# mlvlab/UP-NeRF

Hardware: AMD Instinct MI355X
Metric: training rays/sec (higher is better)
Workload: dtype f32 (f16x3 emulated: 3 fp16 MFMAs per product, fp32 accumulate); 1 GPU; BASELINE.json configs[1]: Brandenburg Gate shape, 4096 rays/GPU/step, 64 coarse + 128 fine samples, two 8x256 fields + candidate/colour heads + TransientNet + appearance/candidate embeddings (763 images), pose optimisation ON, full step incl. both Adam updates; rays_per_gpu=4096, n_images=763, N_samples=64, N_importance=128, parallelism=dp1, field=f16x3

## Files before the change

include/upnerf_hip.h:

```cpp
#ifndef UPNERF_HIP_H
#define UPNERF_HIP_H

#include <stdint.h>

#ifdef __cplusplus
extern "C" {
#endif

#define UPNERF_ABI_VERSION 11
#define UPNERF_EINVAL (-1)
#define UPNERF_EUNSUP (-2)

#ifndef UPNERF_TILE_ROWS
#define UPNERF_TILE_ROWS 64
#endif
#define UPNERF_X0 64
#define UPNERF_AUXK 80
#define UPNERF_CK 16
#define UPNERF_MAX_D 8

int upnerf_abi_version(void);

int upnerf_pose_rays_fwd(int R, const float* se3, const float* c2w, const float* dirs,
                         float* rays_o, float* rays_d, void* stream);
// ... 164 lines not shown
  const float* x0; const float* h; const float* g1; const float* g2; const float* r1;
  const uint64_t* hmask;
  float* gmax;
  float* gz_h;
  float* gz_e;
  float* gz_g1; float* gz_g2;
  float* gz_r1;
  float* dpre_sig_s;
  float* dpre_sig_c;
  float* dpre_rgb;
  float* dxyz;
  const void* PT16;
  const int32_t* wexp;
  int32_t planes;
  int32_t tile_rows;
  uint16_t* gz16;
  int32_t* gzexp;
  void* xs;
  float* tile_part;
  int32_t gz_rg_ld;
  int32_t reserved_;
  const float* wnorm;
  uint16_t* gz_rg16;
  int32_t* gzrgexp;
  uint16_t* gz_g2_16;
  int32_t* gzg2exp;
  uint8_t* gz_lo8;
  int64_t rows_capacity;
} upnerf_field_bwd_args;

#define UPNERF_TILE_PART_STRIDE 1288
int upnerf_tile_part_finish(int R, int S, const float* tile_part, float* rs_g1, float* rs_r1, float* d_wcsig, float* d_bcsig,
                            float* d_wr2, float* d_br2, float* scratch, void* stream);

#define UPNERF_RR_PART_STRIDE 512
int upnerf_ray_part_finish(int R, int S, const float* tile_part, float* rs_g1, float* rs_r1, void* stream);

int upnerf_field_bwd(const upnerf_layout* L, const upnerf_field_bwd_args* a, void* stream);
int upnerf_field_bwd_f16x3(const upnerf_layout* L, const upnerf_field_bwd_args* a, void* stream);

int upnerf_wgrad(int M, const float* A, int lda, int N, const float* B, int ldb, int K,
                 float* dW, int ldo, float* db, float* slabs, int nsplit, void* stream);

#define UPNERF_MAX_WGRAD_GROUPS 32
typedef struct {
  const float* A;
  const float* B;
  float* dW;
  float* db;
  int32_t M, N, K, lda, ldb, ldo;
} upnerf_wgrad_group;
int upnerf_wgrad_grouped_scratch(const upnerf_wgrad_group* groups, int ngroups, int nsplit);
int upnerf_wgrad_grouped(const upnerf_wgrad_group* groups, int ngroups, float* scratch, int nsplit, void* stream);

typedef struct {
  int32_t R; float beta_min;
  const float* feat;
  const float* t_emb;
  const float* w0; const float* b0;
  const float* w1; const float* b1;
  const float* w2; const float* b2;
  const float* w3; const float* b3;
  const float* wf; const float* bf;
  const float* wt; const float* bt;
  const float* wa; const float* ba;
  const float* wb; const float* bb;
  const float* wr; const float* br;
  float* h;
  float* e;
  float* t;
  float* alpha; float* rgb; float* beta;
  float* spre;
} upnerf_transient_args;
typedef struct {
  const float* d_alpha; const float* d_rgb; const float* d_beta;
  float* dz_heads;
  float* gz_t;
  float* gz_e;
  float* gz_h;
  float* g_temb;
  float* g_feat;
} upnerf_transient_grads;
int upnerf_transient_fwd(const upnerf_transient_args* a, void* stream);
int upnerf_transient_bwd(const upnerf_transient_args* a, const upnerf_transient_grads* g, void* stream);

enum {
  UPNERF_WG_F32 = 0,
  UPNERF_WG_F16_TILE,
  UPNERF_WG_F16_FRAG,
  UPNERF_WG_F24,
  UPNERF_WG_PLANES
};
typedef struct {
  const void* p;
  const void* lo;
  const int32_t* exp;
  int32_t ld, kind;
} upnerf_wgrad_operand;

typedef struct {
  const float* slabs; const float* bslabs;
  float* dW; float* db;
  int32_t N, K, TN, TK, nsplit, ldo, rblocks;
  int32_t n2;
  float* dW2; float* db2;
  int32_t ldo2, pad;
// ... 506 lines not shown
```

upnerf_amd/_lib.py:

```python
from __future__ import annotations

import ctypes as C
import os

import torch

from .pass_plan import (AUXK, CK, RR_PART_STRIDE, TILE_PART_STRIDE, WG_F16_FRAG, WG_F16_TILE, WG_F24, WG_F32,
                        WG_PLANES, X0)

_HERE = os.path.dirname(os.path.abspath(__file__))
LIB_PATH = os.environ.get("UPNERF_LIB") or os.path.join(_HERE, "libupnerf_hip.so")
MAX_D = 8

_fp = C.c_void_p


class Layout(C.Structure):
    _fields_ = [("W", C.c_int32), ("D", C.c_int32), ("skip", C.c_int32),
                ("w", C.c_int32 * MAX_D), ("b", C.c_int32 * MAX_D),
                ("we", C.c_int32), ("be", C.c_int32), ("wsig", C.c_int32), ("bsig", C.c_int32),
                ("wc1", C.c_int32), ("bc1", C.c_int32), ("wc2", C.c_int32), ("bc2", C.c_int32),
                ("wcsig", C.c_int32), ("bcsig", C.c_int32), ("wr1", C.c_int32), ("br1", C.c_int32),
                ("wr2", C.c_int32), ("br2", C.c_int32), ("total", C.c_int32),
                ("t_w", C.c_int32 * MAX_D), ("t_skipx", C.c_int32), ("t_we", C.c_int32), ("t_head", C.c_int32),
# ... 307 lines not shown
    _fields_ = [("R", C.c_int32), ("n_tables", C.c_int32), ("hit", _fp), ("t0", _fp), ("t1", _fp), ("rays", _fp), ("rays_c", _fp),
                ("index", _fp), ("count", _fp), ("scratch", _fp), ("tables", PathTable * PATH_MAX_TABLES)]


class OccScatterArgs(C.Structure):
    _fields_ = [("R", C.c_int32), ("n_hit", C.c_int32), ("background", C.c_float), ("reserved_", C.c_int32), ("index", _fp),
                ("rays", _fp), ("rgb_c", _fp), ("depth_c", _fp), ("rgb", _fp), ("depth", _fp)]


class DensityGradArgs(C.Structure):
    _fields_ = [("M", C.c_int32), ("reserved_", C.c_int32), ("points", _fp), ("P", _fp), ("PT", _fp), ("wk_xyz", C.c_float * 10),
                ("sigma", _fp), ("grad", _fp)]


class NormalCompositeArgs(C.Structure):
    _fields_ = [("R", C.c_int32), ("S", C.c_int32), ("grad", _fp), ("w", _fp), ("normal", _fp)]


class VizNormalsArgs(C.Structure):
    _fields_ = [("H", C.c_int32), ("W", C.c_int32), ("n", _fp), ("rot", _fp), ("rgb", _fp)]


class Rng(C.Structure):
    _fields_ = [("seed", C.c_uint64), ("step", C.c_int32), ("row0", C.c_int32), ("row_stride", C.c_int32), ("step_dev", _fp)]


_i, _f, _p = C.c_int, C.c_float, C.c_void_p
_SIGNATURES = {
    "upnerf_abi_version": [],
    "upnerf_pose_rays_fwd": [_i, _p, _p, _p, _p, _p, _p],
    "upnerf_pose_rays_bwd": [_i, _p, _p, _p, _p, _p, _p, _p],
    "upnerf_sample_coarse": [_i, _i, _p, _p, _p, _f, _i, _p, _p],
    "upnerf_uniform_keyed": [_i, _i, C.c_uint64, _i, _p, _i, _i, _i, _p, _p],
    "upnerf_sample_pdf": [_i, _i, _p, _p, _p, _i, _i, _p, _i, _p],
    "upnerf_sort_rows": [_i, _i, _p, _p],
    "upnerf_sample_coarse_keyed": [_i, _i, _p, _p, C.POINTER(Rng), _f, _i, _p, _p],
    "upnerf_resample_sort": [_i, _i, _p, _p, _i, _i, _p, _i, _p, _i, _i, _p, _i, _i, C.POINTER(Rng), _p, _p],
    "upnerf_ray_aux": [_i, _p, _p, C.POINTER(C.c_float), _p, _p, _p],
    "upnerf_field_fwd": [C.POINTER(Layout), C.POINTER(FieldFwdArgs), _p],
    "upnerf_composite_fwd": [C.POINTER(CompositeFwdArgs), _p],
    "upnerf_composite_bwd": [C.POINTER(CompositeBwdArgs), _p],
    "upnerf_field_bwd": [C.POINTER(Layout), C.POINTER(FieldBwdArgs), _p],
    "upnerf_field_fwd_f16x3": [C.POINTER(Layout), C.POINTER(FieldFwdArgs), _p],
    "upnerf_field_bwd_f16x3": [C.POINTER(Layout), C.POINTER(FieldBwdArgs), _p],
    "upnerf_frag16": [_p, _p, _p, C.POINTER(Frag16Desc), _i, C.POINTER(Frag16Desc), _i, _p, _p, _i, _i, _p, _p],
    "upnerf_wgrad": [_i, _p, _i, _i, _p, _i, _i, _p, _i, _p, _p, _i, _p],
    "upnerf_wgrad16_scratch": [C.POINTER(WgradDesc)],
    "upnerf_wgrad16": [C.POINTER(WgradDesc), C.POINTER(WgradPending), _p],
    "upnerf_wgrad_finish": [_p, _p],
    "upnerf_transient_fwd": [_p, _p],
    "upnerf_transient_bwd": [_p, _p, _p],
    "upnerf_wgrad_grouped_scratch": [C.POINTER(WgradGroup), _i, _i],
    "upnerf_wgrad_grouped": [C.POINTER(WgradGroup), _i, _p, _i, _p],
    "upnerf_vec_wgrad": [_i, _p, _i, _i, _p, _i, _i, _p, _p, _p, _i, _p],
    "upnerf_matvec": [_i, _i, _p, _i, _p, _p, _p, _i, _p],
    "upnerf_matvec_rank1": [_i, _i, _p, _i, _p, _p, _p, _i, _p, _p],
    "upnerf_add_pairs": [C.POINTER(AddPair), _i, _p],
    "upnerf_zero": [_p, C.c_longlong, _p],
    "upnerf_vec_wgrad_frag16": [_i, _p, _i, _i, _p, _p, _i, _p, _p, _p, _i, _p],
    "upnerf_ray_sum": [_i, _i, _p, _i, _p, _p],
    "upnerf_ray_part_finish": [_i, _i, _p, _p, _p, _p],
    "upnerf_tile_part_finish": [_i, _i, _p, _p, _p, _p, _p, _p, _p, _p, _p],
    "upnerf_ray_geom_bwd": [_i, _i, _p, _p, _p, _p, _p],
    "upnerf_pack": [_p, C.POINTER(PackDesc), _i, _i, _p],
    "upnerf_gather_rays": [C.POINTER(GatherRaysArgs), _p],
    "upnerf_embed_bwd": [_i, _i, _i, _p, _p, _p, _p],
    "upnerf_embed_bwd_grouped": [_i, _i, _p, C.POINTER(EmbedGroup), _i, _p],
    "upnerf_embed_fwd_grouped": [_i, _i, _p, C.POINTER(EmbedRowsGroup), _i, _p],
    "upnerf_linear": [_i, _i, _i, _p, _i, _p, _i, _p, _p, _i, _i, _p],
    "upnerf_loss_fwd": [C.POINTER(LossArgs), _p, _p, _p, _p],
    "upnerf_loss_bwd": [C.POINTER(LossArgs), _p, C.POINTER(LossGrads), _p],
    "upnerf_frag_copy": [_p, _p, C.POINTER(FragDesc), _i, _p],
    "upnerf_adam": [C.c_int64, _p, _p, _p, _p, _f, _f, _f, _f, _f, _p, _p],
    "upnerf_adam_gather": [_p, _p, _p, _p, _i, _f, _f, _f, _f, _f, _p, _p],
    "upnerf_set_scalars": [_p, _i, C.POINTER(C.c_float), _p],
    "upnerf_scale_exponents": [_p, _i, _p, _p],
    "upnerf_ssim_scratch": [C.POINTER(SsimArgs)],
    "upnerf_ssim": [C.POINTER(SsimArgs), _p, _p],
    "upnerf_conv2d": [C.POINTER(Conv2dArgs), _p],
    "upnerf_maxpool2d": [C.POINTER(Maxpool2dArgs), _p],
    "upnerf_lpips_dist": [C.POINTER(LpipsDistArgs), _p, _p],
    "upnerf_lpips_scratch": [C.POINTER(LpipsScratchArgs)],
    "upnerf_scene_rays": [C.POINTER(SceneRaysArgs), C.POINTER(SceneImage), _p, _p],
    "upnerf_resize_scratch": [C.POINTER(ResizeArgs)],
    "upnerf_resize_linear": [C.POINTER(ResizeArgs), C.POINTER(ResizeMap), _p, _p],
    "upnerf_viz_minmax_scratch": [C.c_longlong],
    "upnerf_viz_minmax": [_p, C.c_longlong, C.c_longlong, _p, _p, _p],
    "upnerf_viz_depth_scratch": [C.POINTER(VizDepthArgs)],
    "upnerf_viz_depth": [C.POINTER(VizDepthArgs), _p, _p],
    "upnerf_viz_pca_scratch": [C.POINTER(VizPcaArgs)],
    "upnerf_viz_pca": [C.POINTER(VizPcaArgs), _p, _p],
    "upnerf_viz_rgb": [C.POINTER(VizRgbArgs), _p],
    "upnerf_path_poses": [C.POINTER(PathPosesArgs), _p],
    "upnerf_path_rays": [C.POINTER(PathRaysArgs), _p],
    "upnerf_grid_columns": [C.POINTER(GridColumnsArgs), _p],
    "upnerf_mtet_scratch": [_i, _i, _i],
    "upnerf_mtet_count": [C.POINTER(MtetArgs), _p, _p, _p],
    "upnerf_mtet_emit": [C.POINTER(MtetArgs), _p, _p],
    "upnerf_occ_words": [_i, _i, _i],
    "upnerf_occ_build_scratch": [_i, _i, _i],
    "upnerf_occ_build": [C.POINTER(OccBuildArgs), _p],
    "upnerf_occ_spans": [C.POINTER(OccSpansArgs), _p],
    "upnerf_occ_compact_scratch": [_i],
    "upnerf_occ_compact": [C.POINTER(OccCompactArgs), _p],
    "upnerf_occ_scatter": [C.POINTER(OccScatterArgs), _p],
    "upnerf_density_grad": [C.POINTER(Layout), C.POINTER(DensityGradArgs), _p],
# ... 69 lines not shown
```

upnerf_amd/csrc/gemm.hip:

```cpp
#include "common.cuh"
#include "wgrad_host.h"

using namespace upnerf_host;

namespace {

template <int MTW, int NTW>
__device__ __forceinline__ void wgrad_tile(int N, int K, const float* __restrict__ A, int lda,
                                           const float* __restrict__ B, int ldb, float* __restrict__ slab,
                                           float* __restrict__ bslab, int mbeg, int mend, int nblk, int kblk) {
  constexpr int TN = 64 * MTW, TK = 64 * NTW;
  constexpr int A4 = WG_CHUNK * TN / 4 / NTHREADS, B4 = WG_CHUNK * TK / 4 / NTHREADS;
  __shared__ __attribute__((aligned(16))) float As[2][WG_CHUNK * TN];
  __shared__ __attribute__((aligned(16))) float Bs[2][WG_CHUNK * TK];
  const int tid = threadIdx.x, lane = tid & 63, wave = tid >> 6;
  const int li = lane & 31, hh = lane >> 5;
  const int n0 = (wave >> 1) * 32 * MTW, k0 = (wave & 1) * 32 * NTW;
  f32x16 acc[MTW][NTW];
  acc_zero(acc);
  float bsum[MTW];
#pragma unroll
  for (int mt = 0; mt < MTW; ++mt) bsum[mt] = 0.f;

  f32x4 ra[A4 > 0 ? A4 : 1], rb[B4 > 0 ? B4 : 1];
// ... 69 lines not shown
      }
  if (bslab && (wave & 1) == 0) {
#pragma unroll
    for (int mt = 0; mt < MTW; ++mt) {
      const float s = bsum[mt] + __shfl_xor(bsum[mt], 32);
      if (hh == 0) bslab[n0 + 32 * mt + li] = s;
    }
  }
}

template <int MTW, int NTW>
__global__ __launch_bounds__(NTHREADS, 1) void wgrad_kernel(int M, int N, int K, const float* __restrict__ A, int lda,
                                                            const float* __restrict__ B, int ldb,
                                                            float* __restrict__ slabs, float* __restrict__ bslabs,
                                                            int rows_per_split) {
  constexpr int TN = 64 * MTW, TK = 64 * NTW;
  const int split = blockIdx.x;
  const int mbeg = split * rows_per_split;
  const int mend = (mbeg + rows_per_split < M) ? mbeg + rows_per_split : M;
  const size_t blk = ((size_t)split * gridDim.y + blockIdx.y) * gridDim.z + blockIdx.z;
  wgrad_tile<MTW, NTW>(N, K, A, lda, B, ldb, slabs + blk * TN * TK,
                       (bslabs && blockIdx.z == 0) ? bslabs + ((size_t)split * gridDim.y + blockIdx.y) * TN : nullptr, mbeg,
                       mend, blockIdx.y * TN, blockIdx.z * TK);
}

struct WgradGroups {
  upnerf_wgrad_group g[UPNERF_MAX_WGRAD_GROUPS];
  int tile_start[UPNERF_MAX_WGRAD_GROUPS + 1];
  int red_start[UPNERF_MAX_WGRAD_GROUPS + 1];
  int n;
};
#define GT 128

__device__ __forceinline__ int find_group(const int* start, int n, int idx) {
  int g = 0;
  while (g + 1 < n && idx >= start[g + 1]) ++g;
  return g;
}

__global__ __launch_bounds__(NTHREADS, 1) void wgrad_grouped_kernel(WgradGroups T, float* __restrict__ slabs,
                                                                    float* __restrict__ bslabs, int nsplit) {
  const int tile = blockIdx.y, split = blockIdx.x;
  const int gi = find_group(T.tile_start, T.n, tile);
  const upnerf_wgrad_group& G = T.g[gi];
  const int gz = (G.K + GT - 1) / GT, local = tile - T.tile_start[gi], by = local / gz, bz = local - by * gz;
  const int rows = (((G.M + nsplit - 1) / nsplit) + WG_CHUNK - 1) / WG_CHUNK * WG_CHUNK;
  const int mbeg = split * rows;
  const int mend = (mbeg + rows < G.M) ? mbeg + rows : G.M;
  const size_t blk = (size_t)tile * nsplit + split;
  wgrad_tile<2, 2>(G.N, G.K, G.A, G.lda, G.B, G.ldb, slabs + blk * GT * GT,
                   (G.db && bz == 0) ? bslabs + blk * GT : nullptr, mbeg < mend ? mbeg : mend, mend, by * GT, bz * GT);
}

__global__ __launch_bounds__(NTHREADS) void wgrad_grouped_reduce_kernel(WgradGroups T, const float* __restrict__ slabs,
                                                                       const float* __restrict__ bslabs, int nsplit) {
  const int gi = find_group(T.red_start, T.n, blockIdx.x);
  const upnerf_wgrad_group& G = T.g[gi];
  const int b = blockIdx.x - T.red_start[gi];
  const int K4 = G.K >> 2, gz = (G.K + GT - 1) / GT;
  const int q = b * NTHREADS + threadIdx.x;
  if (q < G.N * K4) {
    const int n = q / K4, k = (q - n * K4) * 4;
    const int by = n / GT, bz = k / GT;
    const float* src = slabs + ((size_t)(T.tile_start[gi] + by * gz + bz) * nsplit) * GT * GT + (size_t)(n - by * GT) * GT +
                       (k - bz * GT);
    f32x4 s0 = {0.f, 0.f, 0.f, 0.f}, s1 = s0, s2 = s0, s3 = s0;
    int sp = 0;
    for (; sp + 4 <= nsplit; sp += 4) {
      const f32x4 a = *(const f32x4*)&src[(size_t)sp * GT * GT], c = *(const f32x4*)&src[(size_t)(sp + 1) * GT * GT];
      const f32x4 d = *(const f32x4*)&src[(size_t)(sp + 2) * GT * GT], e = *(const f32x4*)&src[(size_t)(sp + 3) * GT * GT];
      s0 += a; s1 += c; s2 += d; s3 += e;
    }
    for (; sp < nsplit; ++sp) s0 += *(const f32x4*)&src[(size_t)sp * GT * GT];
    *(f32x4*)&G.dW[(size_t)n * G.ldo + k] = (s0 + s1) + (s2 + s3);
  }
  if (G.db && q < G.N) {
    const int by = q / GT;
    const float* src = bslabs + ((size_t)(T.tile_start[gi] + by * gz) * nsplit) * GT + (q - by * GT);
    float p0 = 0.f, p1 = 0.f, p2 = 0.f, p3 = 0.f;
    int sp = 0;
    for (; sp + 4 <= nsplit; sp += 4) {
      p0 += src[(size_t)sp * GT]; p1 += src[(size_t)(sp + 1) * GT];
      p2 += src[(size_t)(sp + 2) * GT]; p3 += src[(size_t)(sp + 3) * GT];
    }
    for (; sp < nsplit; ++sp) p0 += src[(size_t)sp * GT];
    G.db[q] = (p0 + p1) + (p2 + p3);
  }
}

__global__ __launch_bounds__(RED_THREADS) void wgrad_reduce_kernel(upnerf_wgrad_pending P) {
  __shared__ f32x4 part[RED_RG][64];
  wgrad_reduce_body(blockIdx.x, threadIdx.x, P, part);
}

template <int K>
__global__ __launch_bounds__(NTHREADS) void vec_wgrad_kernel(int M, const float* __restrict__ v, int ldv, int nvec,
                                                            const float* __restrict__ X, int ldx,
                                                            float* __restrict__ part, int rows_per_split) {
  constexpr int CPR = K / 4, RG = NTHREADS / CPR;
  __shared__ float red[RG][3][K + 4];
  const int tid = threadIdx.x, c4 = tid % CPR, rg = tid / CPR, split = blockIdx.x;
  const int mbeg = split * rows_per_split;
  const int mend = (mbeg + rows_per_split < M) ? mbeg + rows_per_split : M;
  f32x4 acc[3];
  float bacc[3] = {0.f, 0.f, 0.f};
#pragma unroll
  for (int c = 0; c < 3; ++c) acc[c] = f32x4{0.f, 0.f, 0.f, 0.f};
  constexpr int U = 8;
  for (int m = mbeg + rg; m < mend; m += U * RG) {
    f32x4 x[U];
    float vv[U][3];
#pragma unroll
    for (int u = 0; u < U; ++u) {
      const int mm = m + u * RG;
      const bool ok = mm < mend;
      const int mc = ok ? mm : mend - 1;
      x[u] = NT_LOAD((const f32x4*)&X[(size_t)mc * ldx + 4 * c4]);
#pragma unroll
      for (int c = 0; c < 3; ++c) vv[u][c] = (c < nvec) ? v[(size_t)mc * ldv + c] : 0.f;
      if (!ok) {
        x[u] = f32x4{0.f, 0.f, 0.f, 0.f};
#pragma unroll
        for (int c = 0; c < 3; ++c) vv[u][c] = 0.f;
      }
    }
#pragma unroll
    for (int u = 0; u < U; ++u)
#pragma unroll
      for (int c = 0; c < 3; ++c) {
        acc[c].x += vv[u][c] * x[u].x; acc[c].y += vv[u][c] * x[u].y;
        acc[c].z += vv[u][c] * x[u].z; acc[c].w += vv[u][c] * x[u].w;
        bacc[c] += vv[u][c];
      }
  }
#pragma unroll
  for (int c = 0; c < 3; ++c) {
    *(f32x4*)&red[rg][c][4 * c4] = acc[c];
    if (c4 == 0) red[rg][c][K] = bacc[c];
  }
// ... 523 lines not shown
#pragma unroll
        for (int u = 0; u < 8; ++u) {
          const int m = m0 + 16 * u;
          const int mc = m < M ? m : M - 1;
          a[u] = A[(size_t)mc * lda + k];
          xv[u] = m < M ? x[mc] : 0.0f;
        }
#pragma unroll
        for (int u = 0; u < 8; ++u) s += a[u] * xv[u];
        if (R1) {
          const float vk = v1[k];
#pragma unroll
          for (int u = 0; u < 8; ++u) {
            const int m = m0 + 16 * u;
            if (m < M) R1[(size_t)m * ldr + k] += xv[u] * vk;
          }
        }
      }
    }
    part[p][c] = s;
    __syncthreads();
    if (p == 0 && k < K) {
      float t = 0.0f;
#pragma unroll
      for (int q = 0; q < 16; ++q) t += part[q][c];
      y[k] = t + (add ? add[k] : 0.0f);
    }
    return;
  }
  const int m = blockIdx.x * 4 + (threadIdx.x >> 6), lane = threadIdx.x & 63;
  if (m >= M) return;
  float s = 0.0f;
  for (int k = lane; k < K; k += 64) s += A[(size_t)m * lda + k] * x[k];
#pragma unroll
  for (int d = 32; d >= 1; d >>= 1) s += __shfl_xor(s, d);
  if (lane == 0) y[m] = s + (add ? add[m] : 0.0f);
}
extern "C" int upnerf_matvec(int M, int K, const float* A, int lda, const float* x, const float* add, float* y, int trans,
                             void* stream) {
  if (M <= 0 || K <= 0 || !A || !x || !y || lda < K) return UPNERF_EINVAL;
  const int blocks = trans ? (K + 15) / 16 : (M + 3) / 4;
  hipLaunchKernelGGL(matvec_kernel, dim3(blocks), dim3(256), 0, (hipStream_t)stream, M, K, A, lda, x, add, y, trans);
  return (int)hipGetLastError();
}

extern "C" int upnerf_matvec_rank1(int M, int K, const float* A, int lda, const float* x, float* y, float* R, int ldr, const float* v,
                                   void* stream) {
  if (M <= 0 || K <= 0 || !A || !x || !y || !R || !v || lda < K || ldr < K) return UPNERF_EINVAL;
  hipLaunchKernelGGL(matvec_kernel, dim3((K + 15) / 16), dim3(256), 0, (hipStream_t)stream, M, K, A, lda, x, (const float*)nullptr, y, 1, R,
                     ldr, v);
  return (int)hipGetLastError();
}

extern "C" int upnerf_wgrad_grouped_scratch(const upnerf_wgrad_group* groups, int ngroups, int nsplit) {
  if (!groups || ngroups <= 0 || ngroups > UPNERF_MAX_WGRAD_GROUPS || nsplit <= 0) return UPNERF_EINVAL;
  long long tiles = 0;
  for (int j = 0; j < ngroups; ++j)
    tiles += (long long)((groups[j].N + GT - 1) / GT) * ((groups[j].K + GT - 1) / GT);
  const long long n = tiles * nsplit * (GT * GT + GT);
  return n > 0x7fffffffLL ? UPNERF_EUNSUP : (int)n;
}

extern "C" int upnerf_wgrad_grouped(const upnerf_wgrad_group* groups, int ngroups, float* scratch, int nsplit,
                                    void* stream) {
  if (!groups || ngroups <= 0 || ngroups > UPNERF_MAX_WGRAD_GROUPS || !scratch || nsplit <= 0) return UPNERF_EINVAL;
  WgradGroups T;
  T.n = ngroups;
  T.tile_start[0] = T.red_start[0] = 0;
  for (int j = 0; j < ngroups; ++j) {
    const upnerf_wgrad_group& q = groups[j];
    if (!q.A || !q.B || !q.dW || q.M <= 0 || q.N <= 0 || q.K <= 0 || (q.N & 3) || (q.K & 3) || (q.lda & 3) || (q.ldb & 3) ||
        (q.ldo & 3))
      return UPNERF_EINVAL;
    T.g[j] = q;
    T.tile_start[j + 1] = T.tile_start[j] + ((q.N + GT - 1) / GT) * ((q.K + GT - 1) / GT);
    int rb = (q.N * (q.K / 4) + NTHREADS - 1) / NTHREADS;
    if (rb * NTHREADS < q.N) rb = (q.N + NTHREADS - 1) / NTHREADS;
    T.red_start[j + 1] = T.red_start[j] + rb;
  }
  const int tiles = T.tile_start[ngroups];
  float* bslabs = scratch + (size_t)tiles * nsplit * GT * GT;
  hipStream_t st = (hipStream_t)stream;
  hipLaunchKernelGGL(wgrad_grouped_kernel, dim3(nsplit, tiles), dim3(NTHREADS), 0, st, T, scratch, bslabs, nsplit);
  int rc = (int)hipGetLastError();
  if (rc) return rc;
  hipLaunchKernelGGL(wgrad_grouped_reduce_kernel, dim3(T.red_start[ngroups]), dim3(NTHREADS), 0, st, T, scratch, bslabs,
                     nsplit);
  return (int)hipGetLastError();
}

extern "C" int upnerf_vec_wgrad(int M, const float* v, int ldv, int nvec, const float* X, int ldx, int K, float* dw,
                                float* dbv, float* scratch, int nsplit, void* stream) {
  if (M <= 0 || nvec <= 0 || nvec > 4 || K <= 0 || K > 256 || !v || !X || !dw || !scratch || nsplit <= 0)
    return UPNERF_EINVAL;
  hipStream_t st = (hipStream_t)stream;
  const int rows = (M + nsplit - 1) / nsplit;
  if (nvec > 3 || (ldx & 3)) return UPNERF_EINVAL;
  if (K == 256) hipLaunchKernelGGL(vec_wgrad_kernel<256>, dim3(nsplit), dim3(NTHREADS), 0, st, M, v, ldv, nvec, X, ldx, scratch, rows);
  else if (K == 128) hipLaunchKernelGGL(vec_wgrad_kernel<128>, dim3(nsplit), dim3(NTHREADS), 0, st, M, v, ldv, nvec, X, ldx, scratch, rows);
  else if (K == 64) hipLaunchKernelGGL(vec_wgrad_kernel<64>, dim3(nsplit), dim3(NTHREADS), 0, st, M, v, ldv, nvec, X, ldx, scratch, rows);
  else if (K == 32) hipLaunchKernelGGL(vec_wgrad_kernel<32>, dim3(nsplit), dim3(NTHREADS), 0, st, M, v, ldv, nvec, X, ldx, scratch, rows);
  else return UPNERF_EUNSUP;
  int rc = (int)hipGetLastError();
  if (rc) return rc;
  const int total = nvec * (K + 1);
  hipLaunchKernelGGL(vec_wgrad_reduce_kernel, dim3((total + 255) / 256), dim3(256), 0, st, nvec, K, nsplit, scratch, dw,
                     dbv);
  return (int)hipGetLastError();
}

#define TP_STRIDE UPNERF_TILE_PART_STRIDE
#define TP_WCOLS 520
#define TP_NS 128
namespace {
__device__ __forceinline__ void tile_part_rays_body(int idx, int which, int R, int S, const float* __restrict__ part,
                                                    float* __restrict__ rs_g1, float* __restrict__ rs_r1) {
  float* __restrict__ out = which == 0 ? rs_g1 : rs_r1;
  if (idx >= R * 32 || !out) return;
  const int r = idx >> 5, g = idx & 31;
  const long long b = (long long)r * S, e = b + S - 1;
  const int t0 = (int)(b / 64), t1 = (int)(e / 64);
  const int base = TP_WCOLS + (which == 0 ? 0 : 384) + 4 * g;
  f32x4 s = {0.f, 0.f, 0.f, 0.f};
  for (int t = t0; t <= t1; ++t) {
    const int j = r - (int)(((long long)t * 64) / S);
    s += *(const f32x4*)&part[(size_t)t * TP_STRIDE + base + 128 * j];
  }
  *(f32x4*)&out[(size_t)r * 128 + 4 * g] = s;
}
// ... 277 lines not shown
```

upnerf_amd/ops.py:

```python
from __future__ import annotations

import contextlib
import ctypes as C
import os
from typing import Dict, NamedTuple, Optional, Tuple

import torch
import torch.nn.functional as F

from . import _lib
from ._lib import check, lib, ptr, stream

_WS: Dict[Tuple[str, int], torch.Tensor] = {}


class KernelTimer:

    def __init__(self):
        self.enabled = False
        self.only = None
        self.records = {}

    def run(self, name: str, fn, units: int = 0):
        if not self.enabled or (self.only is not None and name not in self.only):
            return fn()
        e0, e1 = torch.cuda.Event(enable_timing=True), torch.cuda.Event(enable_timing=True)
        e0.record()
        out = fn()
        e1.record()
        self.records.setdefault(name, []).append((e0, e1, units))
        return out

    def reset(self):
        self.records = {}

    def summary(self):
        torch.cuda.synchronize()
        out = {}
        for name, evs in self.records.items():
            ms = [a.elapsed_time(b) for a, b, _ in evs]
            out[name] = dict(launches=len(ms), total_ms=sum(ms), avg_ms=sum(ms) / len(ms),
                             units_per_launch=sum(u for _, _, u in evs) / len(evs))
        return out


TIMER = KernelTimer()


def workspace(tag: str, numel: int, device) -> torch.Tensor:
    key = (tag, device.index if device.index is not None else torch.cuda.current_device())
    t = _WS.get(key)
    if t is None or t.numel() < numel:
        t = torch.empty(max(numel, 1), device=device, dtype=torch.float32)
        _WS[key] = t
    return t


def nsplit_for(M: int) -> int:
    return max(1, min(256, M // 64))


def wgrad_into(M: int, A: torch.Tensor, lda: int, N: int, B: torch.Tensor, ldb: int, K: int, dW_ptr: int, ldo: int,
               db_ptr: Optional[int], device, a_off: int = 0, b_off: int = 0):
    ns = nsplit_for(M)
    ws = workspace("wgrad", ns * (256 * 256 + 256), device)
    rc = TIMER.run(f"wgrad_{N}x{K}", lambda: lib.upnerf_wgrad(M, A.data_ptr() + 4 * a_off, lda, N,
                                                              B.data_ptr() + 4 * b_off, ldb, K, dW_ptr, ldo, db_ptr,
                                                              ptr(ws), ns, stream()), units=M)
    check(rc, "upnerf_wgrad")


def wgrad_blocks_into(M: int, A: torch.Tensor, lda: int, N: int, B: torch.Tensor, ldb: int, K: int, dW_ptr: int, ldo: int,
                      db_ptr: Optional[int], device, a_off: int = 0, b_off: int = 0):
    g = _lib.WgradGroup(A=A.data_ptr() + 4 * a_off, B=B.data_ptr() + 4 * b_off, dW=dW_ptr, db=db_ptr, M=M, N=N, K=K, lda=lda,
                        ldb=ldb, ldo=ldo)
    arr = (_lib.WgradGroup * 1)(g)
    nsplit = max(1, min(_DeferredWgrads.NSPLIT, M // 64))
    n = lib.upnerf_wgrad_grouped_scratch(arr, 1, nsplit)
    if n < 0:
        check(n, "upnerf_wgrad_grouped_scratch")
    ws = workspace("wgrad_blocks", n, device)
    check(TIMER.run(f"wgrad_blocks_{N}x{K}", lambda: lib.upnerf_wgrad_grouped(arr, 1, ptr(ws), nsplit, stream())),
          "upnerf_wgrad_grouped")


class _DeferredWgrads:

    enabled = __import__("os").environ.get("UPNERF_DEFER_WGRADS", "1") != "0"
    check_adopted = __import__("os").environ.get("UPNERF_CHECK_DEFERRED", "0") == "1"
    MAX_M = 16384
    NSPLIT = 64

    def __init__(self):
        self.groups, self.keep, self.owners = [], [], []

    def clear(self):
        self.groups, self.keep, self.owners = [], [], []

    def add(self, M, gy, lda, N, x, ldb, K, gw, gb, owners=()):
        self.owners += [(p, t.data_ptr()) for p, t in owners if t is not None]
        torch.autograd.Variable._execution_engine.queue_callback(self.flush)
        self.groups.append(_lib.WgradGroup(A=gy.data_ptr(), B=x.data_ptr(), dW=gw.data_ptr(),
                                           db=None if gb is None else gb.data_ptr(), M=M, N=N, K=K, lda=lda, ldb=ldb,
                                           ldo=K))
        self.keep.append((gy, x, gw.untyped_storage(), None if gb is None else gb.untyped_storage()))
        if len(self.groups) == _lib.MAX_WGRAD_GROUPS:
            self._launch()

    def _launch(self):
        groups, self.groups = self.groups, []
        keep, self.keep = self.keep, []
        owners, self.owners = self.owners, []
        if not groups:
            return
        if self.check_adopted:
            for p, addr in owners:
                if p.grad is None or p.grad.data_ptr() != addr:
                    raise RuntimeError("deferred weight gradient was not adopted by its parameter (autograd copied or "
                                       "summed the still empty buffer)")
        arr = (_lib.WgradGroup * len(groups))(*groups)
        n = lib.upnerf_wgrad_grouped_scratch(arr, len(groups), self.NSPLIT)
        if n < 0:
            check(n, "upnerf_wgrad_grouped_scratch")
        ws = workspace("wgrad_grouped", n, keep[0][0].device)
        check(TIMER.run("wgrad_grouped", lambda: lib.upnerf_wgrad_grouped(arr, len(groups), ptr(ws), self.NSPLIT,
                                                                          stream())), "upnerf_wgrad_grouped")

    def flush(self):
        self._launch()


DEFERRED_WGRADS = _DeferredWgrads()


def can_adopt(p) -> bool:
    return (p is not None and isinstance(p, torch.nn.Parameter) and p.is_leaf and p.grad is None
            and not p._backward_hooks and not getattr(p, "_post_accumulate_grad_hooks", None))


_DEFER_USES: Dict[int, list] = {}


def _defer_token(*leaves):
    toks = []
    for p in leaves:
        if p is not None:
            t = _DEFER_USES.setdefault(id(p), [0])
            t[0] += 1
            toks.append(t)
    return toks


def reset_deferred():
    DEFERRED_WGRADS.clear()
    DEFERRED_EMBEDS.items = []
    _DEFER_USES.clear()


def scale_exponents(A: torch.Tensor, B: torch.Tensor) -> torch.Tensor:
    amax = torch.stack([A.abs().amax(), B.abs().amax()]).clamp_min(1e-30)
    return (14 - torch.ceil(torch.log2(amax))).to(torch.int32)


class WgOp(NamedTuple):
    t: torch.Tensor
    ld: int
    kind: int = _lib.WG_F32
    exp: Optional[torch.Tensor] = None
    lo: Optional[torch.Tensor] = None
    off: int = 0

    def c(self):
        p = self.t.data_ptr() + 4 * self.off if self.kind == _lib.WG_F32 else ptr(self.t)
        return _lib.WgradOperand(p=p, lo=ptr(self.lo), exp=ptr(self.exp), ld=self.ld, kind=self.kind)


_WG_TIMER = {_lib.WG_F32: "wgrad16", _lib.WG_F16_TILE: "wgrad16p", _lib.WG_F16_FRAG: "wgrad16p", _lib.WG_F24: "wgrad24p",
             _lib.WG_PLANES: "wgrad16hl"}

# ... 333 lines not shown
```

upnerf_amd/transient_net.py:

```python
from __future__ import annotations

import ctypes as C
import os

import torch
import torch.nn as nn
import torch.nn.functional as F

from . import _lib
from ._lib import check, lib, ptr, stream
from .ops import _DeferredWgrads, embed_rows, hip_linear, workspace

FUSED = os.environ.get("UPNERF_TRANSIENT_FUSED", "1") != "0"


class _TransientFn(torch.autograd.Function):

    NAMES = ("w0", "b0", "w1", "b1", "w2", "b2", "w3", "b3", "wf", "bf", "wt", "bt", "wa", "ba", "wb", "bb", "wr", "br")

    @staticmethod
    def forward(ctx, beta_min, feat, t_emb, *params):
        R, dev = feat.shape[0], feat.device
        feat, t_emb = feat.detach().contiguous(), t_emb.detach().contiguous()
        p = [q.detach().contiguous() for q in params]
        e = lambda *s: torch.empty(*s, device=dev, dtype=torch.float32)
        h, ee, t = e(4, R, 256), e(R, 256), e(R, 128)
        alpha, rgb, beta, spre = e(R, 1), e(R, 3), e(R, 1), e(R)
        a = _lib.TransientArgs(R=R, beta_min=float(beta_min), feat=ptr(feat), t_emb=ptr(t_emb), h=ptr(h), e=ptr(ee), t=ptr(t),
                               alpha=ptr(alpha), rgb=ptr(rgb), beta=ptr(beta), spre=ptr(spre),
                               **{n: ptr(q) for n, q in zip(_TransientFn.NAMES, p)})
        check(lib.upnerf_transient_fwd(C.byref(a), stream()), "upnerf_transient_fwd")
        ctx.args, ctx.keep = a, (feat, t_emb, p, h, ee, t, alpha, rgb, beta, spre)
        ctx.set_materialize_grads(False)
        return alpha, rgb, beta

    @staticmethod
    def backward(ctx, d_alpha, d_rgb, d_beta):
        a = ctx.args
        feat, t_emb, p, h, ee, t, alpha, rgb, beta, spre = ctx.keep
        R, dev = feat.shape[0], feat.device
        e = lambda *s: torch.empty(*s, device=dev, dtype=torch.float32)
        c = lambda x: None if x is None else x.contiguous()
        d_alpha, d_rgb, d_beta = c(d_alpha), c(d_rgb), c(d_beta)
        dz, gz_t, gz_e, gz_h = e(R, 8), e(R, 128), e(R, 256), e(4, R, 256)
        g_feat = e(R, 384) if ctx.needs_input_grad[1] else None
        g_temb = e(R, 128) if ctx.needs_input_grad[2] else None
        g = _lib.TransientGrads(d_alpha=ptr(d_alpha), d_rgb=ptr(d_rgb), d_beta=ptr(d_beta), dz_heads=ptr(dz), gz_t=ptr(gz_t),
                                gz_e=ptr(gz_e), gz_h=ptr(gz_h), g_temb=ptr(g_temb), g_feat=ptr(g_feat))
        check(lib.upnerf_transient_bwd(C.byref(a), C.byref(g), stream()), "upnerf_transient_bwd")
        gw = [e(*q.shape) for q in p[:12]]
        hw, ht, hb = e(8, 256), e(8, 128), e(8)
        G = _lib.WgradGroup
        grp = lambda A, lda, N, B, ldb, K, dW, ldo, db: G(A=A, B=B, dW=dW, db=db, M=R, N=N, K=K, lda=lda, ldb=ldb, ldo=ldo)
        groups = [grp(ptr(gz_h[0]), 256, 256, ptr(feat), 384, 384, ptr(gw[0]), 384, ptr(gw[1]))]
        for l in (1, 2, 3):
            groups.append(grp(ptr(gz_h[l]), 256, 256, ptr(h[l - 1]), 256, 256, ptr(gw[2 * l]), 256, ptr(gw[2 * l + 1])))
        groups += [grp(ptr(gz_e), 256, 256, ptr(h[3]), 256, 256, ptr(gw[8]), 256, ptr(gw[9])),
                   grp(ptr(gz_t), 128, 128, ptr(ee), 256, 256, ptr(gw[10]), 384, ptr(gw[11])),
                   grp(ptr(gz_t), 128, 128, ptr(t_emb), 128, 128, gw[10].data_ptr() + 4 * 256, 384, None),
                   grp(ptr(dz), 8, 8, ptr(h[3]), 256, 256, ptr(hw), 256, ptr(hb)),
                   grp(ptr(dz), 8, 8, ptr(t), 128, 128, ptr(ht), 128, None)]
        arr = (G * len(groups))(*groups)
        ns = max(1, min(_DeferredWgrads.NSPLIT, R // 64))
        n = lib.upnerf_wgrad_grouped_scratch(arr, len(groups), ns)
        if n < 0:
            check(n, "upnerf_wgrad_grouped_scratch")
        ws = workspace("wgrad_transient", n, dev)
        check(lib.upnerf_wgrad_grouped(arr, len(groups), ptr(ws), ns, stream()), "upnerf_wgrad_grouped")
        grads = gw + [hw[0:1], hb[0:1], ht[1:2], hb[1:2], ht[2:5], hb[2:5]]
        return (None, g_feat, g_temb) + tuple(grads)


class TransientNet(nn.Module):
    def __init__(self, N_images, beta_min=0.1, trasient_dim=128, feat_dim=384):
        super().__init__()
        self.beta_min, self.trasient_dim, self.feat_dim = beta_min, trasient_dim, feat_dim
        self.embedding_t = nn.Embedding(N_images, trasient_dim)
        self.feat_encoder = nn.Sequential(nn.Linear(feat_dim, 256), nn.ReLU(), nn.Linear(256, 256), nn.ReLU(),
                                          nn.Linear(256, 256), nn.ReLU(), nn.Linear(256, 256), nn.ReLU())
        self.final_encoder = nn.Linear(256, 256)
        self.t_encoder = nn.Sequential(nn.Linear(256 + trasient_dim, 128), nn.ReLU())
        self.alpha_layer = nn.Sequential(nn.Linear(256, 1), nn.Sigmoid())
        self.beta_layer = nn.Sequential(nn.Linear(128, 1), nn.Softplus())
        self.rgb_layer = nn.Sequential(nn.Linear(128, 3), nn.Sigmoid())

    def _fused_params(self):
        mods = (self.feat_encoder[0], self.feat_encoder[2], self.feat_encoder[4], self.feat_encoder[6], self.final_encoder,
                self.t_encoder[0], self.alpha_layer[0], self.beta_layer[0], self.rgb_layer[0])
        return [q for m in mods for q in (m.weight, m.bias)]

    def forward(self, feat, ts):
        if FUSED and feat.is_cuda and self.feat_dim == 384 and self.trasient_dim == 128 and feat.dtype == torch.float32:
            t_emb = embed_rows(self.embedding_t, ts, defer_grad=True)
            alpha, rgb, beta = _TransientFn.apply(self.beta_min, feat, t_emb, *self._fused_params())
            return {"alpha": alpha, "rgb": rgb, "beta": beta}
        lin = lambda m, x, relu=False: hip_linear(x, m.weight, m.bias, relu, defer_wgrad=True)
        h = feat
        for i in (0, 2, 4, 6):
            h = lin(self.feat_encoder[i], h, True)
        e = lin(self.final_encoder, h)
        t = lin(self.t_encoder[0], torch.cat([e, embed_rows(self.embedding_t, ts, defer_grad=True)], -1), True)
        alpha = torch.sigmoid(lin(self.alpha_layer[0], h))
        rgb = torch.sigmoid(lin(self.rgb_layer[0], t))
        beta = F.softplus(lin(self.beta_layer[0], t)) * alpha + self.beta_min
        return {"alpha": alpha, "rgb": rgb, "beta": beta}
```

Baseline: 258,900 rays/s.

## Fuse grouped weight-gradient GEMM and split-K reduction into one kernel with tickets

Replaces the two-kernel grouped wgrad (per-split slab writes followed by a separate reduce kernel) with one kernel. Each tile now runs only 1 or 4 blocks, and each block loops over several M-splits, accumulating in registers. An atomic ticket counter per tile lets the last-arriving block sum the few partial slabs and write dW/db. This removes a kernel launch and most of the slab traffic, and allows non-multiple-of-4 N/K through store_quad. The cost is far less parallelism across M (only up to 4 blocks per tile), a dependence on the counter being reset to zero, and a scratch buffer that must start zeroed.

Result: no change. 259,600 rays/s (median of 6 runs) (+0.3%).

```diff
diff --git a/include/upnerf_hip.h b/include/upnerf_hip.h
--- a/include/upnerf_hip.h
+++ b/include/upnerf_hip.h
@@ -240,6 +240,7 @@
 } upnerf_wgrad_group;
 int upnerf_wgrad_grouped_scratch(const upnerf_wgrad_group* groups, int ngroups, int nsplit);
 int upnerf_wgrad_grouped(const upnerf_wgrad_group* groups, int ngroups, float* scratch, int nsplit, void* stream);
+int upnerf_wgrad_grouped_fused(const upnerf_wgrad_group* groups, int ngroups, float* scratch, int nsplit, void* stream);
 
 typedef struct {
   int32_t R; float beta_min;
diff --git a/upnerf_amd/_lib.py b/upnerf_amd/_lib.py
--- a/upnerf_amd/_lib.py
+++ b/upnerf_amd/_lib.py
@@ -383,6 +383,7 @@
     "upnerf_transient_bwd": [_p, _p, _p],
     "upnerf_wgrad_grouped_scratch": [C.POINTER(WgradGroup), _i, _i],
     "upnerf_wgrad_grouped": [C.POINTER(WgradGroup), _i, _p, _i, _p],
+    "upnerf_wgrad_grouped_fused": [C.POINTER(WgradGroup), _i, _p, _i, _p],
     "upnerf_vec_wgrad": [_i, _p, _i, _i, _p, _i, _i, _p, _p, _p, _i, _p],
     "upnerf_matvec": [_i, _i, _p, _i, _p, _p, _p, _i, _p],
     "upnerf_matvec_rank1": [_i, _i, _p, _i, _p, _p, _p, _i, _p, _p],
diff --git a/upnerf_amd/csrc/gemm.hip b/upnerf_amd/csrc/gemm.hip
--- a/upnerf_amd/csrc/gemm.hip
+++ b/upnerf_amd/csrc/gemm.hip
@@ -145,12 +145,22 @@
                    (G.db && bz == 0) ? bslabs + blk * GT : nullptr, mbeg < mend ? mbeg : mend, mend, by * GT, bz * GT);
 }
 
+__device__ __forceinline__ void store_quad(float* __restrict__ dst, const f32x4 v, int left) {
+  if (left >= 4) {
+    *(f32x4*)dst = v;
+  } else {
+#pragma unroll
+    for (int j = 0; j < 3; ++j)
+      if (j < left) dst[j] = v[j];
+  }
+}
+
 __global__ __launch_bounds__(NTHREADS) void wgrad_grouped_reduce_kernel(WgradGroups T, const float* __restrict__ slabs,
                                                                        const float* __restrict__ bslabs, int nsplit) {
   const int gi = find_group(T.red_start, T.n, blockIdx.x);
   const upnerf_wgrad_group& G = T.g[gi];
   const int b = blockIdx.x - T.red_start[gi];
-  const int K4 = G.K >> 2, gz = (G.K + GT - 1) / GT;
+  const int K4 = (G.K + 3) >> 2, gz = (G.K + GT - 1) / GT;
   const int q = b * NTHREADS + threadIdx.x;
   if (q < G.N * K4) {
     const int n = q / K4, k = (q - n * K4) * 4;
@@ -165,7 +175,7 @@
       s0 += a; s1 += c; s2 += d; s3 += e;
     }
     for (; sp < nsplit; ++sp) s0 += *(const f32x4*)&src[(size_t)sp * GT * GT];
-    *(f32x4*)&G.dW[(size_t)n * G.ldo + k] = (s0 + s1) + (s2 + s3);
+    store_quad(&G.dW[(size_t)n * G.ldo + k], (s0 + s1) + (s2 + s3), G.K - k);
   }
   if (G.db && q < G.N) {
     const int by = q / GT;
@@ -178,6 +188,142 @@
     }
     for (; sp < nsplit; ++sp) p0 += src[(size_t)sp * GT];
     G.db[q] = (p0 + p1) + (p2 + p3);
+  }
+}
+
+
+#define FT 64
+#define FUSED_CTR 1024
+struct WgradGroupsFused {
+  upnerf_wgrad_group g[UPNERF_MAX_WGRAD_GROUPS];
+  int tile_start[UPNERF_MAX_WGRAD_GROUPS + 1];
+  int n;
+};
+__global__ __launch_bounds__(NTHREADS, 2) void wgrad_grouped_fused_kernel(WgradGroupsFused T, float* scratch, int nsplit, int ncls) {
+  __shared__ __attribute__((aligned(16))) float As[2][WG_CHUNK * FT];
+  __shared__ __attribute__((aligned(16))) float Bs[2][WG_CHUNK * FT];
+  const int tile = blockIdx.y, cls = blockIdx.x;
+  const int gi = find_group(T.tile_start, T.n, tile);
+  const upnerf_wgrad_group& G = T.g[gi];
+  const int M = G.M, N = G.N, K = G.K;
+  const int gz = (K + FT - 1) / FT, local = tile - T.tile_start[gi], by = local / gz, bz = local - by * gz;
+  const int nblk = by * FT, kblk = bz * FT;
+  const int rows = (((M + nsplit - 1) / nsplit) + WG_CHUNK - 1) / WG_CHUNK * WG_CHUNK;
+  const int n4 = ncls == 4 ? nsplit >> 2 : 0;
+  const int nsp = n4 + (cls == 0 ? nsplit - 4 * n4 : 0);
+  const int tid = threadIdx.x, lane = tid & 63, wave = tid >> 6;
+  const int li = lane & 31, hh = lane >> 5;
+  const int n0 = (wave >> 1) * 32, k0 = (wave & 1) * 32;
+  const float* __restrict__ A = G.A;
+  const float* __restrict__ B = G.B;
+  const int lda = G.lda, ldb = G.ldb;
+
+  struct Cur { int i, mc, mend; };
+  auto enter = [&](Cur& c) {
+    const int sp = c.i < n4 ? cls + 4 * c.i : 4 * n4 + (c.i - n4);
+    const long long b = (long long)sp * rows;
+    c.mc = b < M ? (int)b : M;
+    c.mend = c.mc + rows < M ? c.mc + rows : M;
+  };
+  auto seek = [&](Cur& c) {
+    while (c.i < nsp && c.mc >= c.mend) {
+      if (++c.i < nsp) enter(c);
+    }
+  };
+  f32x4 ra[2], rb[2];
+  auto gload = [&](const Cur& c) {
+#pragma unroll
+    for (int q = 0; q < 2; ++q) {
+      const int idx = tid + q * NTHREADS, row = idx >> 4, c4 = idx & 15;
+      const int m = c.mc + row;
+      ra[q] = (m < c.mend && nblk + 4 * c4 < N) ? *(const f32x4*)&A[(size_t)m * lda + nblk + 4 * c4] : f32x4{0.f, 0.f, 0.f, 0.f};
+      rb[q] = (m < c.mend && kblk + 4 * c4 < K) ? *(const f32x4*)&B[(size_t)m * ldb + kblk + 4 * c4] : f32x4{0.f, 0.f, 0.f, 0.f};
+    }
+  };
+  f32x16 acc, tot;
+#pragma unroll
+  for (int r = 0; r < 16; ++r) acc[r] = tot[r] = 0.f;
+  float bsum = 0.f, btot = 0.f;
+  Cur cur{0, 0, 0}, nxt;
+  if (nsp > 0) enter(cur);
+  seek(cur);
+  if (cur.i < nsp) gload(cur);
+  int buf = 0;
+  while (cur.i < nsp) {
+#pragma unroll
+    for (int q = 0; q < 2; ++q) {
+      *(f32x4*)&As[buf][(tid + q * NTHREADS) * 4] = ra[q];
+      *(f32x4*)&Bs[buf][(tid + q * NTHREADS) * 4] = rb[q];
+    }
+    __syncthreads();
+    nxt = cur;
+    nxt.mc += WG_CHUNK;
+    seek(nxt);
+    if (nxt.i < nsp) gload(nxt);
+    const float* as = As[buf] + hh * FT + n0 + li;
+    const float* bs = Bs[buf] + hh * FT + k0 + li;
+#pragma unroll
+    for (int mm = 0; mm < WG_CHUNK; mm += 2) {
+      const float av = as[mm * FT], bv = bs[mm * FT];
+      bsum += av;
+      acc = __builtin_amdgcn_mfma_f32_32x32x2f32(av, bv, acc, 0, 0, 0);
+    }
+    if (nxt.i != cur.i) {
+#pragma unroll
+      for (int r = 0; r < 16; ++r) {
+        tot[r] += acc[r];
+        acc[r] = 0.f;
+      }
+      btot += bsum + __shfl_xor(bsum, 32);
+      bsum = 0.f;
+    }
+    cur = nxt;
+    buf ^= 1;
+  }
+  unsigned int* ctr = (unsigned int*)scratch + tile;
+  float* cslabs = scratch + FUSED_CTR + (size_t)tile * ncls * (FT * FT + FT);
+  float* bslabs = cslabs + (size_t)ncls * FT * FT;
+  {
+    float* slab = cslabs + (size_t)cls * FT * FT;
+#pragma unroll
+    for (int r = 0; r < 16; ++r) slab[(n0 + (r & 3) + 8 * (r >> 2) + 4 * hh) * FT + k0 + li] = tot[r];
+    if (G.db && bz == 0 && (wave & 1) == 0 && hh == 0) bslabs[cls * FT + n0 + li] = btot;
+  }
+  asm volatile("s_waitcnt vmcnt(0)" ::: "memory");
+  __syncthreads();
+  if (tid == 0) {
+    __builtin_amdgcn_fence(__ATOMIC_RELEASE, "agent");
+    asm volatile("s_waitcnt vmcnt(0)" ::: "memory");
+    const unsigned int t = __hip_atomic_fetch_add(ctr, 1u, __ATOMIC_RELAXED, __HIP_MEMORY_SCOPE_AGENT);
+    const bool last = t == (unsigned int)(ncls - 1);
+    if (last) {
+      __hip_atomic_store(ctr, 0u, __ATOMIC_RELAXED, __HIP_MEMORY_SCOPE_AGENT);
+      __builtin_amdgcn_fence(__ATOMIC_ACQUIRE, "agent");
+      asm volatile("s_waitcnt vmcnt(0)" ::: "memory");
+    }
+    As[0][0] = last ? 1.f : 0.f;
+  }
+  __syncthreads();
+  if (As[0][0] == 0.f) return;
+  const f32x4 z4 = {0.f, 0.f, 0.f, 0.f};
+#pragma unroll
+  for (int j = 0; j < FT * FT / 4 / NTHREADS; ++j) {
+    const int q = tid + j * NTHREADS, nl = q >> 4, kq = (q & 15) * 4;
+    const int n = nblk + nl, k = kblk + kq;
+    if (n < N && k < K) {
+      const float* src = cslabs + nl * FT + kq;
+      const f32x4 s0 = *(const f32x4*)src;
+      const f32x4 s1 = ncls == 4 ? *(const f32x4*)&src[FT * FT] : z4;
+      const f32x4 s2 = ncls == 4 ? *(const f32x4*)&src[2 * FT * FT] : z4;
+      const f32x4 s3 = ncls == 4 ? *(const f32x4*)&src[3 * FT * FT] : z4;
+      store_quad(&G.dW[(size_t)n * G.ldo + k], (s0 + s1) + (s2 + s3), K - k);
+    }
+  }
+  if (G.db && bz == 0 && tid < FT && nblk + tid < N) {
+    const float p0 = bslabs[tid];
+    const float p1 = ncls == 4 ? bslabs[FT + tid] : 0.f, p2 = ncls == 4 ? bslabs[2 * FT + tid] : 0.f;
+    const float p3 = ncls == 4 ? bslabs[3 * FT + tid] : 0.f;
+    G.db[nblk + tid] = (p0 + p1) + (p2 + p3);
   }
 }
 
@@ -807,13 +953,44 @@
   return (int)hipGetLastError();
 }
 
+static long long fused_tiles(const upnerf_wgrad_group* groups, int ngroups) {
+  long long tiles = 0;
+  for (int j = 0; j < ngroups; ++j) tiles += (long long)((groups[j].N + FT - 1) / FT) * ((groups[j].K + FT - 1) / FT);
+  return tiles;
+}
+
 extern "C" int upnerf_wgrad_grouped_scratch(const upnerf_wgrad_group* groups, int ngroups, int nsplit) {
   if (!groups || ngroups <= 0 || ngroups > UPNERF_MAX_WGRAD_GROUPS || nsplit <= 0) return UPNERF_EINVAL;
   long long tiles = 0;
   for (int j = 0; j < ngroups; ++j)
     tiles += (long long)((groups[j].N + GT - 1) / GT) * ((groups[j].K + GT - 1) / GT);
-  const long long n = tiles * nsplit * (GT * GT + GT);
+  long long n = tiles * nsplit * (GT * GT + GT);
+  const long long ftiles = fused_tiles(groups, ngroups);
+  const long long nf = FUSED_CTR + ftiles * (nsplit >= 4 ? 4 : 1) * (FT * FT + FT);
+  if (nf > n) n = nf;
   return n > 0x7fffffffLL ? UPNERF_EUNSUP : (int)n;
+}
+
+static bool bad_group_strides(const upnerf_wgrad_group& q) {
+  return (q.lda & 3) || (q.ldb & 3) || (q.ldo & 3) || q.lda < ((q.N + 3) & ~3) || q.ldb < ((q.K + 3) & ~3) || q.ldo < q.K;
+}
+
+extern "C" int upnerf_wgrad_grouped_fused(const upnerf_wgrad_group* groups, int ngroups, float* scratch, int nsplit, void* stream) {
+  if (!groups || ngroups <= 0 || ngroups > UPNERF_MAX_WGRAD_GROUPS || !scratch || nsplit <= 0) return UPNERF_EINVAL;
+  WgradGroupsFused T;
+  T.n = ngroups;
+  T.tile_start[0] = 0;
+  for (int j = 0; j < ngroups; ++j) {
+    const upnerf_wgrad_group& q = groups[j];
+    if (!q.A || !q.B || !q.dW || q.M <= 0 || q.N <= 0 || q.K <= 0 || bad_group_strides(q)) return UPNERF_EINVAL;
+    T.g[j] = q;
+    T.tile_start[j + 1] = T.tile_start[j] + ((q.N + FT - 1) / FT) * ((q.K + FT - 1) / FT);
+  }
+  const int tiles = T.tile_start[ngroups];
+  if (tiles > FUSED_CTR) return UPNERF_EUNSUP;
+  const int ncls = nsplit >= 4 ? 4 : 1;
+  hipLaunchKernelGGL(wgrad_grouped_fused_kernel, dim3(ncls, tiles), dim3(NTHREADS), 0, (hipStream_t)stream, T, scratch, nsplit, ncls);
+  return (int)hipGetLastError();
 }
 
 extern "C" int upnerf_wgrad_grouped(const upnerf_wgrad_group* groups, int ngroups, float* scratch, int nsplit,
@@ -824,12 +1001,10 @@
   T.tile_start[0] = T.red_start[0] = 0;
   for (int j = 0; j < ngroups; ++j) {
     const upnerf_wgrad_group& q = groups[j];
-    if (!q.A || !q.B || !q.dW || q.M <= 0 || q.N <= 0 || q.K <= 0 || (q.N & 3) || (q.K & 3) || (q.lda & 3) || (q.ldb & 3) ||
-        (q.ldo & 3))
-      return UPNERF_EINVAL;
+    if (!q.A || !q.B || !q.dW || q.M <= 0 || q.N <= 0 || q.K <= 0 || bad_group_strides(q)) return UPNERF_EINVAL;
     T.g[j] = q;
     T.tile_start[j + 1] = T.tile_start[j] + ((q.N + GT - 1) / GT) * ((q.K + GT - 1) / GT);
-    int rb = (q.N * (q.K / 4) + NTHREADS - 1) / NTHREADS;
+    int rb = (q.N * ((q.K + 3) / 4) + NTHREADS - 1) / NTHREADS;
     if (rb * NTHREADS < q.N) rb = (q.N + NTHREADS - 1) / NTHREADS;
     T.red_start[j + 1] = T.red_start[j] + rb;
   }
diff --git a/upnerf_amd/ops.py b/upnerf_amd/ops.py
--- a/upnerf_amd/ops.py
+++ b/upnerf_amd/ops.py
@@ -56,6 +56,24 @@
     return t
 
 
+def ticket_workspace(tag: str, numel: int, device) -> torch.Tensor:
+    key = (tag, device.index if device.index is not None else torch.cuda.current_device())
+    t = _WS.get(key)
+    if t is None or t.numel() < numel:
+        t = torch.zeros(max(numel, 1), device=device, dtype=torch.float32)
+        _WS[key] = t
+    return t
+
+
+def wgrad_grouped(arr, ngroups: int, nsplit: int, tag: str, device, timer: Optional[str] = None):
+    n = lib.upnerf_wgrad_grouped_scratch(arr, ngroups, nsplit)
+    if n < 0:
+        check(n, "upnerf_wgrad_grouped_scratch")
+    ws = ticket_workspace(tag, n, device)
+    call = lambda: lib.upnerf_wgrad_grouped_fused(arr, ngroups, ptr(ws), nsplit, stream())
+    check(TIMER.run(timer, call) if timer else call(), "upnerf_wgrad_grouped_fused")
+
+
 def nsplit_for(M: int) -> int:
     return max(1, min(256, M // 64))
 
@@ -76,12 +94,7 @@
                         ldb=ldb, ldo=ldo)
     arr = (_lib.WgradGroup * 1)(g)
     nsplit = max(1, min(_DeferredWgrads.NSPLIT, M // 64))
-    n = lib.upnerf_wgrad_grouped_scratch(arr, 1, nsplit)
-    if n < 0:
-        check(n, "upnerf_wgrad_grouped_scratch")
-    ws = workspace("wgrad_blocks", n, device)
-    check(TIMER.run(f"wgrad_blocks_{N}x{K}", lambda: lib.upnerf_wgrad_grouped(arr, 1, ptr(ws), nsplit, stream())),
-          "upnerf_wgrad_grouped")
+    wgrad_grouped(arr, 1, nsplit, "wgrad_blocks_fused", device, f"wgrad_blocks_{N}x{K}")
 
 
 class _DeferredWgrads:
@@ -119,12 +132,7 @@
                     raise RuntimeError("deferred weight gradient was not adopted by its parameter (autograd copied or "
                                        "summed the still empty buffer)")
         arr = (_lib.WgradGroup * len(groups))(*groups)
-        n = lib.upnerf_wgrad_grouped_scratch(arr, len(groups), self.NSPLIT)
-        if n < 0:
-            check(n, "upnerf_wgrad_grouped_scratch")
-        ws = workspace("wgrad_grouped", n, keep[0][0].device)
-        check(TIMER.run("wgrad_grouped", lambda: lib.upnerf_wgrad_grouped(arr, len(groups), ptr(ws), self.NSPLIT,
-                                                                          stream())), "upnerf_wgrad_grouped")
+        wgrad_grouped(arr, len(groups), self.NSPLIT, "wgrad_grouped_fused", keep[0][0].device, "wgrad_grouped")
 
     def flush(self):
         self._launch()
diff --git a/upnerf_amd/transient_net.py b/upnerf_amd/transient_net.py
--- a/upnerf_amd/transient_net.py
+++ b/upnerf_amd/transient_net.py
@@ -9,7 +9,7 @@
 
 from . import _lib
 from ._lib import check, lib, ptr, stream
-from .ops import _DeferredWgrads, embed_rows, hip_linear, workspace
+from .ops import _DeferredWgrads, embed_rows, hip_linear, wgrad_grouped
 
 FUSED = os.environ.get("UPNERF_TRANSIENT_FUSED", "1") != "0"
 
@@ -62,11 +62,7 @@
                    grp(ptr(dz), 8, 8, ptr(t), 128, 128, ptr(ht), 128, None)]
         arr = (G * len(groups))(*groups)
         ns = max(1, min(_DeferredWgrads.NSPLIT, R // 64))
-        n = lib.upnerf_wgrad_grouped_scratch(arr, len(groups), ns)
-        if n < 0:
-            check(n, "upnerf_wgrad_grouped_scratch")
-        ws = workspace("wgrad_transient", n, dev)
-        check(lib.upnerf_wgrad_grouped(arr, len(groups), ptr(ws), ns, stream()), "upnerf_wgrad_grouped")
+        wgrad_grouped(arr, len(groups), ns, "wgrad_transient_fused", dev)
         grads = gw + [hw[0:1], hb[0:1], ht[1:2], hb[1:2], ht[2:5], hb[2:5]]
         return (None, g_feat, g_temb) + tuple(grads)
 
```
